# huggingface/parler-tts

Measured on NVIDIA H100. Metric: audio codec tokens/sec (all codebooks), higher is better.
Workload: dtype bf16

## Files before the change

### parler_tts_b200/csrc/sample_core.cuh

```cuda
#pragma once
#include <cfloat>
#include "common.cuh"
#include "kernels.h"

namespace ptts {

__device__ __forceinline__ uint32_t fkey(float f) {
  uint32_t u = __float_as_uint(f);
  return (u & 0x80000000u) ? ~u : (u | 0x80000000u);
}

__device__ __forceinline__ void philox_round(uint32_t (&c)[4], uint32_t k0, uint32_t k1) {
  const uint32_t hi0 = __umulhi(0xD2511F53u, c[0]), lo0 = 0xD2511F53u * c[0];
  const uint32_t hi1 = __umulhi(0xCD9E8D57u, c[2]), lo1 = 0xCD9E8D57u * c[2];
  c[0] = hi1 ^ c[1] ^ k0; c[1] = lo1; c[2] = hi0 ^ c[3] ^ k1; c[3] = lo0;
}
__device__ __forceinline__ float philox_uniform(uint64_t seed, uint32_t row, uint32_t col) {
  uint32_t c[4] = {row, col, 0x5054u, 0x5453u};
  uint32_t k0 = (uint32_t)seed, k1 = (uint32_t)(seed >> 32);
#pragma unroll
  for (int i = 0; i < 10; i++) { philox_round(c, k0, k1); k0 += 0x9E3779B9u; k1 += 0xBB67AE85u; }
  return (float)(c[0] >> 8) * (1.0f / 16777216.0f);
}


constexpr int SMP_WARPS = 8;
constexpr int SMP_THREADS = SMP_WARPS * 32;

constexpr int SMP_MAX_ROWS = 3;
struct SmpScratch {
  float f[2][SMP_MAX_ROWS][SMP_WARPS];
  int i[2][SMP_MAX_ROWS][SMP_WARPS];
  int z[2][SMP_MAX_ROWS][SMP_WARPS];
};
__device__ __forceinline__ SmpScratch& smp_scratch() {
  __shared__ SmpScratch sc;
  return sc;
}
constexpr int SMP_BAN_WORDS = 9 * SMP_THREADS / 32;
__device__ __forceinline__ uint32_t (&smp_bans())[SMP_MAX_ROWS][SMP_BAN_WORDS] {
  __shared__ uint32_t ban[SMP_MAX_ROWS][SMP_BAN_WORDS];
  return ban;
}
struct SmpSeq {
  int last[SMP_MAX_ROWS][PTTS_SEQ_BIAS_MAX];
  float bias[PTTS_SEQ_BIAS_MAX];
};
__device__ __forceinline__ SmpSeq& smp_seq() {
  __shared__ SmpSeq sq;
  return sq;
}
__device__ __forceinline__ bool bitmap_has(const uint32_t* __restrict__ bits, int i) { return (__ldg(bits + (i >> 5)) >> (i & 31)) & 1u; }

template <int ITEMS, int R, bool EXT = false, bool RAGGED = false>
__device__ __forceinline__ void sample_rows_cta(const SampleArgs& p, const ptts_gen_params& g, const int64_t* __restrict__ forced,
                                                int row0, int stride, int n_rows, int cur_len, ptts_sampling_ext x = {},
                                                SampleOut o = {}, ptts_logits_ext lx = {}) {
  static_assert(R >= 1 && R <= SMP_MAX_ROWS, "rows per pass");
  SmpScratch& sc = smp_scratch();
  float (&s_f)[2][SMP_MAX_ROWS][SMP_WARPS] = sc.f;
  int (&s_i)[2][SMP_MAX_ROWS][SMP_WARPS] = sc.i;
  int (&s_z)[2][SMP_MAX_ROWS][SMP_WARPS] = sc.z;
  const int tid = threadIdx.x, lane = tid & 31, warp = tid >> 5;
  int buf = 0;
  auto cta_sum_i = [&](int (&v)[R]) {
#pragma unroll
    for (int r = 0; r < R; r++) {
      const int w = __reduce_add_sync(0xffffffffu, v[r]);
      if (lane == 0) s_i[buf][r][warp] = w;
    }
    __syncthreads();
#pragma unroll
    for (int r = 0; r < R; r++) {
      int a = 0;
#pragma unroll
      for (int w = 0; w < SMP_WARPS; w++) a += s_i[buf][r][w];
      v[r] = a;
    }
    buf ^= 1;
  };
  auto cta_sum_f = [&](float (&v)[R]) {
#pragma unroll
    for (int r = 0; r < R; r++) {
      const float w = warp_sum(v[r]);
      if (lane == 0) s_f[buf][r][warp] = w;
    }
    __syncthreads();
#pragma unroll
    for (int r = 0; r < R; r++) {
      float a = 0.f;
#pragma unroll
      for (int w = 0; w < SMP_WARPS; w++) a += s_f[buf][r][w];
      v[r] = a;
    }
    buf ^= 1;
  };
  auto cta_max_f = [&](float (&v)[R]) {
#pragma unroll
    for (int r = 0; r < R; r++) {
      const float w = warp_max(v[r]);
      if (lane == 0) s_f[buf][r][warp] = w;
    }
    __syncthreads();
#pragma unroll
    for (int r = 0; r < R; r++) {
      float a = s_f[buf][r][0];
#pragma unroll
      for (int w = 1; w < SMP_WARPS; w++) a = fmaxf(a, s_f[buf][r][w]);
      v[r] = a;
    }
    buf ^= 1;
  };

  int row[R];
  bool valid[R];
  int col[R];
  float v[R][ITEMS];
#pragma unroll
  for (int r = 0; r < R; r++) {
    row[r] = row0 + r * stride;
    valid[r] = row[r] < n_rows;
    col[r] = cur_len - ((RAGGED && valid[r]) ? row_shift(p.shift, row[r] / p.K) : 0);
#pragma unroll
    for (int j = 0; j < ITEMS; j++) {
      const int i = tid + SMP_THREADS * j;
      v[r][j] = (valid[r] && i < p.V) ? __ldcg(p.logits + (size_t)row[r] * p.V + i) : -INFINITY;
    }
  }
  auto out_row = [&](float* base, int r) -> float* {
    const int step = cur_len - (g.input_len > 1 ? g.input_len : 1);
    if (base == nullptr || !valid[r] || step < o.first_step || step - o.first_step >= o.n_steps) return nullptr;
    return base + (int64_t)(step - o.first_step) * o.step_stride + (int64_t)row[r] * p.V;
  };
  if constexpr (EXT) {
#pragma unroll
    for (int r = 0; r < R; r++) {
      if (float* dst = out_row(o.logits, r)) {
#pragma unroll
        for (int j = 0; j < ITEMS; j++) {
          const int i = tid + SMP_THREADS * j;
          if (i < p.V) __stcs(dst + i, v[r][j]);
// ... 34 lines not shown
#pragma unroll
  for (int r = 0; r < R; r++) {
    forced_bos[r] = EXT && lx.forced_bos_token_id >= 0 && col[r] == 1;
    const int sh = cur_len - col[r];
    const int begin = lx.begin_index - sh + ((sh > 0 && g.input_len - sh == 1 && lx.forced_bos_token_id >= 0) ? 1 : 0);
    begin_sup[r] = EXT && lx.begin_suppress != nullptr && col[r] == begin;
  }
  if constexpr (EXT) {
    if (lx.n_seq > 0) {
      SmpSeq& sq = smp_seq();
#pragma unroll
      for (int r = 0; r < R; r++) {
        for (int q = tid; q < lx.n_seq; q += SMP_THREADS) {
          const int32_t* e = lx.seq + q * (1 + PTTS_SEQ_BIAS_MAX_LEN);
          const int len = e[0];
          int last = -1;
          if (valid[r] && len >= 2 && len <= PTTS_SEQ_BIAS_MAX_LEN && len <= col[r]) {
            const int64_t* h = p.raw_ids + (size_t)row[r] * p.raw_ld + col[r] - (len - 1);
            bool match = true;
            for (int t = 0; t < len - 1 && match; t++) match = h[t] == e[1 + t];
            if (match) last = e[len];
          }
          sq.last[r][q] = last;
          if (r == 0) sq.bias[q] = lx.seq_bias[q];
        }
      }
      __syncthreads();
    }
  }
#pragma unroll
  for (int r = 0; r < R; r++) {
    const int b = row[r] / p.K, k = row[r] - b * p.K;
    bool mask_eos = false;
    if (cur_len - (g.input_len > 1 ? g.input_len : 1) < g.min_new_tokens) mask_eos = true;
    const bool mask_min = mask_eos;
    bool mask_par = false;
    if (valid[r]) {
      const int par = cur_len & 1;
      int fu = p.first_unf[par * p.B + b];
      const int es = __ldcg(p.eos_seen + fu);
      if (es > 0 && es <= col[r] && fu < b * p.K + p.K - 1) fu++;
      if (k == 0 && tid == 0) p.first_unf[(par ^ 1) * p.B + b] = fu;
      if (row[r] > fu) mask_eos = mask_par = true;
    }
    if (seq_bias || forced_bos[r] || forced_eos || decay || (EXT && lx.remove_invalid_values)) {
      const float mult = decay ? __ldg(lx.decay + cur_len) : 0.f;
#pragma unroll
      for (int j = 0; j < ITEMS; j++) {
        const int i = tid + SMP_THREADS * j;
        if (i >= p.V) continue;
        float y = v[r][j];
        if (seq_bias) {
          float bs = lx.bias1 != nullptr ? __fadd_rn(0.f, __ldg(lx.bias1 + i)) : 0.f;
          for (int q = 0; q < lx.n_seq; q++)
            if (smp_seq().last[r][q] == i) bs = __fadd_rn(bs, smp_seq().bias[q]);
          y = __fadd_rn(y, bs);
        }
        if (bans && ((smp_bans()[r][i >> 5] >> (i & 31)) & 1u)) y = -INFINITY;
        if (mask_min && i == p.eos) y = -INFINITY;
        if (forced_bos[r]) y = (i == lx.forced_bos_token_id) ? 0.f : -INFINITY;
        if (forced_eos) y = (i == lx.forced_eos_token_id) ? 0.f : -INFINITY;
        if (lx.remove_invalid_values) y = (y != y) ? 0.f : (y == INFINITY ? FLT_MAX : (y == -INFINITY ? -FLT_MAX : y));
        if (decay) y = __fadd_rn(y, i == p.eos ? __fmul_rn(fabsf(y), mult) : 0.f);
        if (lx.suppress != nullptr && bitmap_has(lx.suppress, i)) y = -INFINITY;
        if (begin_sup[r] && bitmap_has(lx.begin_suppress, i)) y = -INFINITY;
        if (mask_par && i == p.eos) y = -INFINITY;
        if (g.suppress_special && i >= g.codebook_size) y = -INFINITY;
        v[r][j] = y;
      }
      continue;
    }
#pragma unroll
    for (int j = 0; j < ITEMS; j++) {
      const int i = tid + SMP_THREADS * j;
      if (mask_eos && i == p.eos) v[r][j] = -INFINITY;
      if (g.suppress_special && i >= g.codebook_size) v[r][j] = -INFINITY;
      if constexpr (EXT) {
        if (bans && ((smp_bans()[r][i >> 5] >> (i & 31)) & 1u)) v[r][j] = -INFINITY;
        if (i < p.V && lx.suppress != nullptr && bitmap_has(lx.suppress, i)) v[r][j] = -INFINITY;
        if (i < p.V && begin_sup[r] && bitmap_has(lx.begin_suppress, i)) v[r][j] = -INFINITY;
      }
    }
  }
  int tok[R];
#pragma unroll
  for (int r = 0; r < R; r++) tok[r] = 0;
  const bool renorm = EXT && lx.renormalize_logits;
  float n_max[R], n_log[R];
  if (g.do_sample) {
    if (g.temperature != 1.0f) {
#pragma unroll
      for (int r = 0; r < R; r++)
#pragma unroll
        for (int j = 0; j < ITEMS; j++) v[r][j] = v[r][j] / g.temperature;
    }
    if (g.top_k > 0) {
      const int kk = g.top_k < p.V ? g.top_k : p.V;
      uint32_t key[R][ITEMS];
      uint32_t th[R];
#pragma unroll
      for (int r = 0; r < R; r++) {
        th[r] = 0;
#pragma unroll
        for (int j = 0; j < ITEMS; j++) key[r][j] = (tid + SMP_THREADS * j < p.V) ? fkey(v[r][j]) : 0u;
      }
      for (int bit = 31; bit >= 0; bit--) {
        int cnt[R];
#pragma unroll
        for (int r = 0; r < R; r++) {
          const uint32_t cand = th[r] | (1u << bit);
          cnt[r] = 0;
#pragma unroll
          for (int j = 0; j < ITEMS; j++) cnt[r] += (key[r][j] >= cand) ? 1 : 0;
        }
        cta_sum_i(cnt);
#pragma unroll
        for (int r = 0; r < R; r++)
          if (cnt[r] >= kk) th[r] |= (1u << bit);
      }
#pragma unroll
      for (int r = 0; r < R; r++)
#pragma unroll
        for (int j = 0; j < ITEMS; j++)
          if (fkey(v[r][j]) < th[r]) v[r][j] = -INFINITY;
    }
    float m[R];
#pragma unroll
    for (int r = 0; r < R; r++) {
      m[r] = -INFINITY;
#pragma unroll
      for (int j = 0; j < ITEMS; j++) m[r] = fmaxf(m[r], v[r][j]);
    }
    cta_max_f(m);
    float e[R][ITEMS];
    float s[R];
#pragma unroll
    for (int r = 0; r < R; r++) {
      s[r] = 0.f;
#pragma unroll
      for (int j = 0; j < ITEMS; j++) { e[r][j] = expf(v[r][j] - m[r]); s[r] += e[r][j]; }
    }
    cta_sum_f(s);
    if (g.top_p < 1.0f) {
      uint32_t th[R];
#pragma unroll
      for (int r = 0; r < R; r++) th[r] = 0;
      for (int bit = 31; bit >= 0; bit--) {
        float c[R];
#pragma unroll
        for (int r = 0; r < R; r++) {
          const uint32_t cand = th[r] | (1u << bit);
          c[r] = 0.f;
#pragma unroll
          for (int j = 0; j < ITEMS; j++) c[r] += (fkey(v[r][j]) <= cand) ? e[r][j] : 0.f;
        }
        cta_sum_f(c);
#pragma unroll
        for (int r = 0; r < R; r++)
          if (c[r] <= (1.0f - g.top_p) * s[r]) th[r] |= (1u << bit);
      }
#pragma unroll
      for (int r = 0; r < R; r++) {
        const uint32_t kmax = fkey(m[r]);
        s[r] = 0.f;
#pragma unroll
        for (int j = 0; j < ITEMS; j++) {
          const uint32_t key = fkey(v[r][j]);
          if (key <= th[r] && key != kmax) { v[r][j] = -INFINITY; e[r][j] = 0.f; }
          s[r] += e[r][j];
        }
      }
      cta_sum_f(s);
    }
    if constexpr (EXT) {
      auto drop_where = [&](auto&& remove) {
#pragma unroll
        for (int r = 0; r < R; r++) {
          const float inv = 1.0f / s[r];
          s[r] = 0.f;
#pragma unroll
          for (int j = 0; j < ITEMS; j++) {
            if (remove(r, j, inv)) { v[r][j] = -INFINITY; e[r][j] = 0.f; }
            s[r] += e[r][j];
          }
        }
        cta_sum_f(s);
      };
      auto entropy = [&](float (&ent)[R], float (&lse)[R]) {
#pragma unroll
        for (int r = 0; r < R; r++) {
          lse[r] = m[r] + logf(s[r]);
          ent[r] = 0.f;
#pragma unroll
          for (int j = 0; j < ITEMS; j++)
            if (v[r][j] > -INFINITY) { const float lp = v[r][j] - lse[r]; ent[r] += lp * expf(lp); }
        }
        cta_sum_f(ent);
#pragma unroll
        for (int r = 0; r < R; r++) ent[r] = -ent[r];
      };
      if (x.min_p > 0.f)
        drop_where([&](int r, int j, float inv) { return e[r][j] * inv < x.min_p * inv; });
      if (x.typical_p < 1.0f) {
        float ent[R], lse[R];
        entropy(ent, lse);
        uint32_t key[R][ITEMS], th[R];
#pragma unroll
        for (int r = 0; r < R; r++) {
          th[r] = 0;
#pragma unroll
          for (int j = 0; j < ITEMS; j++) key[r][j] = fkey(v[r][j] > -INFINITY ? fabsf(lse[r] - v[r][j] - ent[r]) : INFINITY);
        }
        for (int bit = 31; bit >= 0; bit--) {
          float c[R];
#pragma unroll
          for (int r = 0; r < R; r++) {
            const uint32_t cand = th[r] | (1u << bit);
            c[r] = 0.f;
#pragma unroll
            for (int j = 0; j < ITEMS; j++) c[r] += (key[r][j] <= cand) ? e[r][j] : 0.f;
          }
          cta_sum_f(c);
#pragma unroll
          for (int r = 0; r < R; r++)
            if (c[r] < x.typical_p * s[r]) th[r] |= (1u << bit);
        }
        drop_where([&](int r, int j, float) { return th[r] != 0xffffffffu && key[r][j] > th[r] + 1u; });
      }
      if (x.epsilon_cutoff > 0.f)
        drop_where([&](int r, int j, float inv) { return e[r][j] * inv < x.epsilon_cutoff && v[r][j] < m[r]; });
      if (x.eta_cutoff > 0.f) {
        float ent[R], lse[R];
        entropy(ent, lse);
        drop_where([&](int r, int j, float inv) {
          return e[r][j] * inv < fminf(x.eta_cutoff, sqrtf(x.eta_cutoff) * expf(-ent[r])) && v[r][j] < m[r];
        });
      }
    }
    float target[R], carry[R];
    int found[R], last_nz[R];
#pragma unroll
    for (int r = 0; r < R; r++) {
      target[r] = philox_uniform(g.seed, (uint32_t)(row[r] + g.row_base), (uint32_t)col[r]) * s[r];
      carry[r] = 0.f; found[r] = -1; last_nz[r] = -1;
    }
#pragma unroll
    for (int j = 0; j < ITEMS; j++) {
      float x[R];
#pragma unroll
      for (int r = 0; r < R; r++) {
        x[r] = e[r][j];
#pragma unroll
        for (int o = 1; o < 32; o <<= 1) {
          const float y = __shfl_up_sync(0xffffffffu, x[r], o);
          if (lane >= o) x[r] += y;
        }
        if (lane == 31) s_f[buf][r][warp] = x[r];
      }
      __syncthreads();
      float tot[R];
#pragma unroll
      for (int r = 0; r < R; r++) {
        float base = carry[r];
        tot[r] = carry[r];
#pragma unroll
        for (int w = 0; w < SMP_WARPS; w++) {
          const float tw = s_f[buf][r][w];
          if (w < warp) base += tw;
          tot[r] += tw;
        }
        const float cum = base + x[r];
        const unsigned hit = __ballot_sync(0xffffffffu, cum > target[r] && e[r][j] > 0.f);
        const unsigned nz = __ballot_sync(0xffffffffu, e[r][j] > 0.f);
        if (lane == 0) {
          s_i[buf][r][warp] = hit ? SMP_THREADS * j + 32 * warp + (__ffs(hit) - 1) : 0x7fffffff;
          s_z[buf][r][warp] = nz ? SMP_THREADS * j + 32 * warp + (31 - __clz(nz)) : -1;
        }
      }
      __syncthreads();
#pragma unroll
      for (int r = 0; r < R; r++) {
        int first = 0x7fffffff, lastz = -1;
#pragma unroll
        for (int w = 0; w < SMP_WARPS; w++) { first = min(first, s_i[buf][r][w]); lastz = max(lastz, s_z[buf][r][w]); }
        if (found[r] < 0 && first != 0x7fffffff) found[r] = first;
        if (lastz >= 0) last_nz[r] = lastz;
        carry[r] = tot[r];
      }
      buf ^= 1;
    }
#pragma unroll
    for (int r = 0; r < R; r++) tok[r] = found[r] >= 0 ? found[r] : last_nz[r];
    if constexpr (EXT) {
#pragma unroll
      for (int r = 0; r < R; r++) {
        if (tok[r] < 0) tok[r] = 0;
        n_max[r] = m[r];
        n_log[r] = logf(s[r]);
      }
    }
  } else {
#pragma unroll
    for (int r = 0; r < R; r++) {
      float m = -INFINITY;
      int mi = 0x7fffffff;
#pragma unroll
      for (int j = 0; j < ITEMS; j++) {
        const int i = tid + SMP_THREADS * j;
        if (i < p.V && (v[r][j] > m || (v[r][j] == m && i < mi))) { m = v[r][j]; mi = i; }
      }
#pragma unroll
      for (int o = 16; o > 0; o >>= 1) {
        const float om = __shfl_xor_sync(0xffffffffu, m, o);
        const int oi = __shfl_xor_sync(0xffffffffu, mi, o);
        if (om > m || (om == m && oi < mi)) { m = om; mi = oi; }
      }
      if (lane == 0) { s_f[buf][r][warp] = m; s_i[buf][r][warp] = mi; }
    }
    __syncthreads();
#pragma unroll
    for (int r = 0; r < R; r++) {
      float m = s_f[buf][r][0];
      int mi = s_i[buf][r][0];
#pragma unroll
      for (int w = 1; w < SMP_WARPS; w++) {
        const float om = s_f[buf][r][w];
        const int oi = s_i[buf][r][w];
        if (om > m || (om == m && oi < mi)) { m = om; mi = oi; }
      }
      tok[r] = mi;
    }
    buf ^= 1;
    if (renorm) {
#pragma unroll
      for (int r = 0; r < R; r++) {
        n_max[r] = -INFINITY;
#pragma unroll
        for (int j = 0; j < ITEMS; j++) n_max[r] = fmaxf(n_max[r], v[r][j]);
      }
      cta_max_f(n_max);
#pragma unroll
      for (int r = 0; r < R; r++) {
        n_log[r] = 0.f;
#pragma unroll
        for (int j = 0; j < ITEMS; j++) n_log[r] += expf(v[r][j] - n_max[r]);
      }
      cta_sum_f(n_log);
#pragma unroll
      for (int r = 0; r < R; r++) n_log[r] = logf(n_log[r]);
    }
  }
  if (renorm) {
#pragma unroll
    for (int r = 0; r < R; r++)
#pragma unroll
      for (int j = 0; j < ITEMS; j++) v[r][j] = (v[r][j] - n_max[r]) - n_log[r];
  }
#pragma unroll
  for (int r = 0; r < R; r++) {
    if (!valid[r]) continue;
#pragma unroll
    for (int j = 0; j < ITEMS; j++) {
      const int i = tid + SMP_THREADS * j;
      if (i < p.V) p.scores[(size_t)row[r] * p.V + i] = v[r][j];
    }
    if constexpr (EXT) {
      if (float* dst = out_row(o.scores, r)) {
#pragma unroll
        for (int j = 0; j < ITEMS; j++) {
          const int i = tid + SMP_THREADS * j;
          if (i < p.V) __stcs(dst + i, v[r][j]);
        }
      }
    }
  }
  int my_tok = 0, my_row = 0, my_col = 0;
  bool my_valid = false;
#pragma unroll
  for (int r = 0; r < R; r++)
    if (tid == r) { my_tok = tok[r]; my_row = row[r]; my_valid = valid[r]; my_col = col[r]; }
  if (tid < R && my_valid) {
    const int b = my_row / p.K, k = my_row - b * p.K;
    int t = my_tok;
    if (forced != nullptr) t = (int)forced[my_row];
    if (!t_unf) t = p.pad;
    p.raw_ids[(size_t)my_row * p.raw_ld + my_col] = t;
    if (t == p.eos && t_es == 0) p.eos_seen[my_row] = my_col + 1;
    const int new_len = cur_len + 1;
    const int done = (t == p.eos) || (new_len >= g.max_length);
    const int still_unfinished = t_unf && !done;
    p.unfinished[my_row] = still_unfinished;
    const int sh = cur_len - my_col;
    const int Lb = g.max_length - sh, nb = g.input_len - sh;
    int nxt = t;
    if (Lb >= 2 * p.K - 1) {
      const bool is_bos = my_col <= k;
      const bool is_pad = (my_col - k) >= (Lb - p.K + 1);
      if (is_bos || is_pad) nxt = (is_bos ? p.bos : 0) + (is_pad ? p.pad : 0);
      else if (nb > 1 && my_col - nb < k) nxt = (int)p.prefix_cells[(size_t)my_row * (p.K - 1) + (my_col - nb)];
    }
    p.cur_ids[my_row] = nxt;
    if (still_unfinished) atomicAdd(&p.ctrl->n_unfinished, 1);
  }
  __syncthreads();
}

template <int ITEMS>
__device__ __forceinline__ void sample_row_cta(const SampleArgs& p, const ptts_gen_params& g, const int64_t* __restrict__ forced,
                                               int row, int cur_len) {
  sample_rows_cta<ITEMS, 1>(p, g, forced, row, 0, row + 1, cur_len);
}

template <int ITEMS, bool RAGGED = false>
__device__ __forceinline__ void sample_all_rows_cta(const SampleArgs& p, const ptts_gen_params& g, int cta, int n_ctas, int n_rows, int cur_len) {
  if (n_rows <= n_ctas) {
    if (cta < n_rows) sample_rows_cta<ITEMS, 1, false, RAGGED>(p, g, nullptr, cta, n_ctas, n_rows, cur_len);
  } else {
    for (int row0 = cta; row0 < n_rows; row0 += 3 * n_ctas) sample_rows_cta<ITEMS, 3, false, RAGGED>(p, g, nullptr, row0, n_ctas, n_rows, cur_len);
  }
}

}
```

### parler_tts_b200/csrc/step2.cu

```cuda
#include "attn_core.cuh"
#include "common.cuh"
#include "kernels.h"
#include "ln_stats.cuh"
#include "sample_core.cuh"
#include "ptx.cuh"
#include "step.h"
#include "step_common.cuh"
#include <type_traits>

namespace ptts {
namespace cl {

constexpr int C = 2;
constexpr int V = 8;
constexpr int THREADS = 256;
constexpr int ROWS = 32;
constexpr int HROWS = 8;
constexpr int ATT_SMEM = attn_decode_smem_per_warp<bf16>();
constexpr int PROF_STRIDE = 16;
constexpr int QMAX = 6;
constexpr int OFF_STATS = 256, OFF_PART = 512, OFF_RES = 2560, OFF_CVEC = 3584;
constexpr int HDR = 5632;
constexpr int WB_BYTES = 65536;
constexpr int R_OFF = HDR + 2 * WB_BYTES;
constexpr int R_BYTES = 92160;
constexpr int QKV_OFF = R_BYTES - 2048;
constexpr int SMEM_BYTES = R_OFF + R_BYTES;
static_assert(SMEM_BYTES + 1024 <= 227 * 1024, "cluster step kernel shared memory");
static_assert(ROWS * (1024 / 2 + 8) * 2 + V * (256 + ROWS * 34 * 4) <= R_BYTES, "fc1 plan");
static_assert(HROWS * (1024 / 2 + 8) * 2 + V * C * (32 + 4 * 96 * 4) <= QKV_OFF, "QKV plan");
constexpr int ATT_STAGE = 2 * 32 * HD * 2;
constexpr int ATT_REST = ATT_SMEM - ATT_STAGE;
constexpr int ATT_S0_QKV = 34 * 1024;
constexpr int ATT_S0_QC = QKV_OFF - V * ATT_STAGE;
constexpr int ATT_S0_WB = WB_BYTES - ATT_STAGE;
static_assert(HROWS * (1024 / 2 + 8) * 2 + V * C * (32 + 4 * 96 * 4) <= ATT_S0_QKV && ATT_S0_QKV + 6 * ATT_STAGE <= QKV_OFF, "attention plan: QKV stages in R");
static_assert(HROWS * (1024 / 2 + 8) * 2 + V * C * (32 + 4 * 32 * 4) <= ATT_S0_QC, "attention plan: q_cross stages in R");
static_assert(2 * ATT_REST <= ATT_S0_QC && 2 * ATT_REST <= ATT_S0_QKV && 6 * ATT_REST <= ATT_S0_WB, "attention plan: second stages");
static_assert(6 * 8 * (1024 / 2) * 2 <= ATT_S0_WB && 16384 + 4 * 128 * 4 <= ATT_S0_WB, "attention plan: QKV weight jobs, out-proj job + pair merge");
static_assert(ROWS * (4096 / 4 + 8) * 2 + V * (256 + ROWS * 8 * 4) <= R_BYTES, "fc2 plan");

__device__ __forceinline__ void mbar_wait(uint64_t* bar, uint32_t parity, int what) {
  uint32_t ok, spins = 0;
  do {
    ok = mbar_try_wait_cluster(bar, parity);
    if (!ok && ++spins > (1u << 22)) { printf("ptts: cluster step mbarrier timeout (cta %d, barrier kind %d)\n", (int)blockIdx.x, what); __trap(); }
  } while (!ok);
}
__device__ __forceinline__ void st_async(uint32_t dst_cluster_addr, float v, uint32_t bar_cluster_addr) {
  asm volatile("st.async.shared::cluster.mbarrier::complete_tx::bytes.b32 [%0], %1, [%2];"
               ::"r"(dst_cluster_addr), "r"(__float_as_uint(v)), "r"(bar_cluster_addr) : "memory");
}
__device__ __forceinline__ void st_async(uint32_t dst_cluster_addr, float2 v, uint32_t bar_cluster_addr) {
  asm volatile("st.async.shared::cluster.mbarrier::complete_tx::bytes.v2.f32 [%0], {%1, %2}, [%3];"
               ::"r"(dst_cluster_addr), "f"(v.x), "f"(v.y), "r"(bar_cluster_addr) : "memory");
}
__device__ __forceinline__ uint32_t mapa(uint32_t addr, uint32_t rank) { uint32_t r; asm volatile("mapa.shared::cluster.u32 %0, %1, %2;" : "=r"(r) : "r"(addr), "r"(rank)); return r; }
__device__ __forceinline__ uint32_t cluster_rank() { uint32_t r; asm volatile("mov.u32 %0, %%cluster_ctarank;" : "=r"(r)); return r; }
__device__ __forceinline__ void cluster_arrive() { asm volatile("barrier.cluster.arrive.release.aligned;" ::: "memory"); }
__device__ __forceinline__ void cluster_wait() { asm volatile("barrier.cluster.wait.acquire.aligned;" ::: "memory"); }
__device__ __forceinline__ void cluster_arrive_reuse() { asm volatile("barrier.cluster.arrive.relaxed.aligned;" ::: "memory"); }

__host__ __device__ __forceinline__ int kslice(int kt) { return (kt & 7) >> 2; }
__host__ __device__ __forceinline__ int klocal(int kt) { return ((kt >> 3) << 2) | (kt & 3); }
__host__ __device__ __forceinline__ int kglobal(int rank, int lk) { return ((lk >> 2) << 3) | (rank << 2) | (lk & 3); }

template <int QN, int MT, bool STATS, bool ACC = false>
__device__ __forceinline__ void mma_slice(float (&out)[2][6][4], RowStatFrag& rst, const bf16* xs, int apitch, const uint4* wb, int KT, int kt0,
                                          int kt_end, int lrow, int lcol) {
  float acc[MT][QN][4];
#pragma unroll
  for (int a = 0; a < MT; a++)
#pragma unroll
    for (int j = 0; j < QN; j++)
#pragma unroll
      for (int e = 0; e < 4; e++) acc[a][j][e] = ACC ? out[a][j][e] : 0.f;
  for (int kt = kt0; kt < kt_end; kt += 4) {
    uint32_t a[MT][2][4];
#pragma unroll
    for (int mt = 0; mt < MT; mt++)
#pragma unroll
      for (int j = 0; j < 2; j++) ldmatrix_x4(a[mt][j], xs + (size_t)(mt * 16 + lrow) * apitch + kt * 32 + j * 16 + lcol);
    if (STATS) {
#pragma unroll
      for (int mt = 0; mt < MT; mt++) { row_stat_mma(rst, mt, a[mt][0]); row_stat_mma(rst, mt, a[mt][1]); }
    }
#pragma unroll
    for (int j = 0; j < QN; j++) {
      const uint4 w = wb[((size_t)j * KT + kt) * 32];
#pragma unroll
      for (int mt = 0; mt < MT; mt++) {
        mma_bf16_16816(acc[mt][j], a[mt][0], w.x, w.y);
        mma_bf16_16816(acc[mt][j], a[mt][1], w.z, w.w);
      }
    }
  }
#pragma unroll
  for (int mt = 0; mt < MT; mt++)
#pragma unroll
    for (int j = 0; j < QN; j++)
#pragma unroll
      for (int e = 0; e < 4; e++) out[mt][j][e] = acc[mt][j][e];
}

enum { PH_QKV = 0, PH_O = 1, PH_QC = 2, PH_OC = 3, PH_FC1 = 4, PH_FC2 = 5 };
constexpr int JOBS_PER_LAYER = 9;
constexpr int QKV_JOBS = 4;

__device__ __forceinline__ bool weight_job(const StepParams& p, int j, int cta, int rank, const char*& src, uint32_t& bytes) {
  const int nl = JOBS_PER_LAYER * p.L;
  if (j < nl) {
    const int l = j / JOBS_PER_LAYER, jl = j - JOBS_PER_LAYER * l;
    const int ph = jl < QKV_JOBS ? 0 : jl - (QKV_JOBS - 1);
    const int64_t idx = (ph == PH_QKV || ph == PH_QC) ? (int64_t)(cta >> 3) * C + rank : (int64_t)cta;
    const int64_t sz = p.lay.cp_slice[ph];
    bytes = (uint32_t)(ph == PH_QKV ? sz / QKV_JOBS : sz);
    src = p.blob + p.lay.layer0 + p.lay.layer_stride * l + p.lay.cp[ph] + idx * sz + (ph == PH_QKV ? jl * (sz / QKV_JOBS) : 0);
    return true;
  }
  const int task = cta + (int)gridDim.x * (j - nl);
  const int ntasks = p.K * p.V / 32;
  if (task >= ntasks) return false;
  bytes = (uint32_t)(4 * p.H * 16);
  src = p.blob + p.lay.heads + (int64_t)task * bytes;
  return true;
}

template <int ITEMS, bool RAGGED>
__global__ void __launch_bounds__(THREADS, 1) decode_step_cluster_kernel(const __grid_constant__ StepParams p) {
  extern __shared__ __align__(128) unsigned char smem[];
  Ctrl* ctrl = p.sa.ctrl;
  if (p.prof != nullptr && blockIdx.x == 0 && threadIdx.x == 0) p.prof[(size_t)(6 * p.L + 2) * PROF_STRIDE + 3] = clock64();
  if (ctrl->active == 0) return;
  int cur_len = ctrl->cur_len;
  const unsigned gen = (unsigned)ctrl->launch_gen;
  int pos = p.P + cur_len - 1;
  const int tid = threadIdx.x, warp = tid >> 5, lane = tid & 31;
  const int H = p.H, F = p.F, B = p.B;
  const int rank = (int)cluster_rank(), peer = rank ^ 1;
  const int cta = (int)blockIdx.x;
  const int cluster = cta >> 1;
  const int head = cluster >> 2, rblk = cluster & 3;
  const int Ks = H / C, KsF = F / 4;
  const int pitch = Ks + 8, pitchF = KsF + 8;
  const int qe = F / p.nh / 64;
  const int dgrp = warp & 1, e4 = warp >> 1;

  uint64_t* abar = reinterpret_cast<uint64_t*>(smem);
  uint64_t* wbar = abar + 1;
  uint64_t* xbar = abar + 3;
  uint64_t* attbars = reinterpret_cast<uint64_t*>(smem + 128);
  float* stats = reinterpret_cast<float*>(smem + OFF_STATS);
  float* part = reinterpret_cast<float*>(smem + OFF_PART);
  float* res_s = reinterpret_cast<float*>(smem + OFF_RES);
  float* cvec = reinterpret_cast<float*>(smem + OFF_CVEC);
  unsigned char* Rg = smem + R_OFF;
  const uint32_t peer_xbar = mapa(smem_u32(xbar), (uint32_t)peer);
  uint32_t par_a = 0, par_w = 0, par_x = 0, att_parity = 0;

  if (tid == 0) {
    mbar_init<1>(abar); mbar_init<1>(&wbar[0]); mbar_init<1>(&wbar[1]); mbar_init<1>(xbar);
    asm volatile("fence.mbarrier_init.release.cluster;" ::: "memory");
  }
  attention_decode_init_warp(attbars + 2 * warp, lane);
  cluster_arrive(); cluster_wait();
  unsigned* const bar_ctr = p.bar + (gen & 1u);
  unsigned bar_target = 0u;
  if (cta == 0 && tid == 0) p.bar[(gen + 1u) & 1u] = 0u;

  const char* blob = p.blob;
  long long* const prof0 = (p.prof != nullptr && cta == 0) ? p.prof : nullptr;
  long long* prof = prof0;
  prof_mark(prof, 0);

  auto issue_weight_job = [&](int j) {
    const char* src; uint32_t bytes;
    if (!weight_job(p, j, cta, rank, src, bytes)) return;
    mbar_expect_tx(&wbar[j & 1], bytes);
    bulk_g2s_evict_first(smem + HDR + (j & 1) * WB_BYTES, src, bytes, &wbar[j & 1]);
  };
  __shared__ int s_next_active;
  const int n_steps = (p.do_sample_phase && p.n_steps > 1 && prof0 == nullptr) ? p.n_steps : 1;
  int unfinished_prev = 0;
#pragma unroll 1
  for (int it = 0; it < n_steps; it++) {
  pos = p.P + cur_len - 1;
  prof = prof0;
  cluster_arrive_reuse();
  if (tid == 0) { issue_weight_job(0); issue_weight_job(1); }

  bf16* const x_img = p.cl_x;
  bf16* const a_img = p.cl_attn;
  bf16* const h_img = p.cl_h;
  const int x_slice_elems = ROWS * pitch, h_slice_elems = ROWS * pitchF;
  auto h_offset = [&](int n) {
    const int lk = klocal(n >> 5), kq = KsF >> 5;
    return (size_t)(2 * kslice(n >> 5) + lk / kq) * h_slice_elems + (lk % kq) * 32 + (n & 31);
  };
  const int xo_slice = kslice(cta >> 2), xo_col = klocal(cta >> 2) * 32 + (cta & 3) * 8;

  {
    const int row = tid >> 3, f = tid & 7, n = cta * 8 + f;
    const float v = row < B ? embed_value(p, row, n, row_pos<RAGGED>(p, row, pos)) : 0.f;
    res_s[row * 8 + f] = v;
    x_img[(size_t)xo_slice * x_slice_elems + row * pitch + xo_col + f] = __float2bfloat16_rn(v);
  }
  prof_mark(prof, 6);
  auto request_slice = [&](const bf16* img_slice, uint32_t bytes) {
    fence_proxy_async_smem();
    mbar_expect_tx(abar, bytes);
    bulk_g2s(Rg, img_slice, bytes, abar);
  };
  auto slice_of = [&](int sub, const bf16*& img, uint32_t& bytes) {
    if (sub == PH_QKV || sub == PH_QC) { img = x_img + (size_t)rank * x_slice_elems + (size_t)(HROWS * rblk) * pitch; bytes = (uint32_t)(HROWS * pitch * 2); }
    else if (sub == PH_O || sub == PH_OC) { img = a_img + (size_t)rank * x_slice_elems; bytes = (uint32_t)(x_slice_elems * 2); }
    else if (sub == PH_FC1) { img = x_img + (size_t)rank * x_slice_elems; bytes = (uint32_t)(x_slice_elems * 2); }
    else { img = h_img + (size_t)(2 * rank) * h_slice_elems; bytes = (uint32_t)(h_slice_elems * 2); }
  };
  {
    const bf16* nimg; uint32_t nbytes;
    slice_of(PH_QKV, nimg, nbytes);
    bar_target = grid_sync(bar_ctr, bar_target, -1, false, nullptr, [&]() { request_slice(nimg, nbytes); });
  }
  prof_mark(prof, 7);

  const int lrow = (lane & 7) + ((lane >> 3) & 1) * 8, lcol = (lane >> 4) * 8;
  const int g = lane >> 2, t4 = lane & 3;
  const int n_phases = 6 * p.L;

  const int att_row = HROWS * rblk + 4 * rank + (warp >> 1);
  const int att_slice = kslice(2 * head), att_col = klocal(2 * head) * 32;

#pragma unroll 1
  for (int ph = 0; ph < n_phases; ph++) {
    const int l = ph / 6, sub = ph - 6 * l;
    prof = prof0 ? prof0 + (size_t)(ph + 1) * PROF_STRIDE : nullptr;
    prof_mark(prof, 0);
    const char* lb = blob + p.lay.layer0 + p.lay.layer_stride * l;
    const bool rowpart = (sub == PH_QKV || sub == PH_QC);
    const bool has_ln = (sub == PH_QKV || sub == PH_QC || sub == PH_FC1);
    const int q = (sub == PH_QKV) ? 6 : (sub == PH_QC ? 2 : (sub == PH_FC1 ? qe : 1));
    const int Nc = 4 * q * 8;
    const int KT = (sub == PH_FC2 ? KsF : Ks) >> 5;
    const int apitch = (sub == PH_FC2) ? pitchF : pitch;
    const int act_bytes = (rowpart ? HROWS : ROWS) * apitch * 2;
    const int RS = (q == 1) ? 8 : 8 * q + 2;
    const int blk = rowpart ? 32 + 4 * 16 * q * 4 : 256 + ROWS * RS * 4;
    unsigned char* const recv = Rg + ((act_bytes + 127) & ~127);
    const uint32_t peer_recv = mapa(smem_u32(recv), (uint32_t)peer);
    const uint32_t xbytes = 4u * (rowpart ? V * 4 * 16 * q + V / 2 * 4 * 2 : V / C * (ROWS * 8 * q + (has_ln ? ROWS * 2 : 0)));
    auto put = [&](int d, uint32_t off, auto v) {
      if (d == rank) *reinterpret_cast<decltype(v)*>(recv + off) = v;
      else st_async(peer_recv + off, v, peer_xbar);
    };
    const int j0 = JOBS_PER_LAYER * l + (sub == 0 ? 0 : sub + QKV_JOBS - 1);
    if (tid == 0) mbar_expect_tx(xbar, xbytes);

    auto att_stage0 = [&]() -> unsigned char* {
      if (sub == PH_QC) return Rg + ATT_S0_QC + warp * ATT_STAGE;
      return warp < 6 ? Rg + ATT_S0_QKV + warp * ATT_STAGE : smem + HDR + (warp - 6) * WB_BYTES + ATT_S0_WB;
    };
    if (rowpart && att_row < B)
      attention_decode_request<bf16>(decode_attn_args(p, l, pos, sub == PH_QC), att_row, head, row_pos<RAGGED>(p, att_row, pos), att_stage0(),
                                     attbars + 2 * warp, lane, warp & 1, 2);

    float cv1 = 0.f, cv2 = 0.f;
    if (has_ln) {
      const float* c1; int ntot;
      if (sub == PH_QKV) { c1 = reinterpret_cast<const float*>(lb + p.lay.c_qkv); ntot = p.qkv_rows; }
      else if (sub == PH_QC) { c1 = reinterpret_cast<const float*>(lb + p.lay.c_qc); ntot = H; }
// ... 132 lines not shown
#pragma unroll
        for (int sv = 0; sv < V; sv++) {
          const float* bp = reinterpret_cast<const float*>(recv + (size_t)sv * blk + 256) + row * RS + f;
          const float2 a = *reinterpret_cast<const float2*>(bp), b2 = *reinterpret_cast<const float2*>(bp + 2);
          v[0] += a.x; v[1] += a.y; v[2] += b2.x; v[3] += b2.y;
        }
#pragma unroll
        for (int e = 0; e < 4; e++) v[e] = apply_act(DT<bf16>::rnd(ln_rstd * (v[e] - ln_mean * cvec[f + e]) + cvec[256 + f + e]), p.act);
        uint2 pk;
        pk.x = att_pack(v[0], v[1]); pk.y = att_pack(v[2], v[3]);
        *reinterpret_cast<uint2*>(h_img + h_offset(cta * 32 + f) + row * pitchF) = pk;
      } else if (row < B) {
        for (int i = 0; i < q; i++) {
          const int f = f0 + 8 * i;
          float v = 0.f;
#pragma unroll
          for (int sv = 0; sv < V; sv++) v += reinterpret_cast<const float*>(recv + (size_t)sv * blk + 256)[row * RS + f];
          if (sub == PH_FC1) {
            v = ln_rstd * (v - ln_mean * cvec[f]) + cvec[256 + f];
            v = apply_act(DT<bf16>::rnd(v), p.act);
            h_img[h_offset(cta * 8 * q + f) + row * pitchF] = __float2bfloat16_rn(v);
          } else {
            v = DT<bf16>::rnd(res_s[row * 8 + f] + DT<bf16>::rnd(v));
            res_s[row * 8 + f] = v;
            x_img[(size_t)xo_slice * x_slice_elems + row * pitch + xo_col + f] = __float2bfloat16_rn(v);
          }
        }
      }
    } else {
      bf16* qkv_s = reinterpret_cast<bf16*>(Rg + QKV_OFF);
      auto gather = [&](auto jw_tag) {
        constexpr int JW = decltype(jw_tag)::value, NC = 4 * JW, QCW = 2 * JW;
        for (int idx = tid; idx < 4 * NC; idx += THREADS) {
          const int r4 = idx / NC, col = idx - r4 * NC;
          const int u = col / JW, cw = (u >> 1) * JW + (col - u * JW);
          float S1 = 0.f, S2 = 0.f;
#pragma unroll
          for (int e = 0; e < V; e++) {
            const float2 x = *reinterpret_cast<const float2*>(recv + (size_t)(8 * (e >> 2) + 2 * (e & 3)) * blk + r4 * 8);
            S1 += x.x; S2 += x.y;
          }
          const float ln_mean = S1 / (float)H;
          const float ln_rstd = rsqrtf(fmaxf(S2 / (float)H - ln_mean * ln_mean, 0.f) + p.eps);
          float v = 0.f;
#pragma unroll
          for (int e = 0; e < V; e++)
            v += reinterpret_cast<const float*>(recv + (size_t)(8 * (e >> 2) + 2 * (e & 3) + (u & 1)) * blk + 32)[r4 * QCW + cw];
          v = ln_rstd * (v - ln_mean * cvec[col]) + cvec[256 + col];
          qkv_s[idx] = __float2bfloat16_rn(v);
        }
      };
      if (sub == PH_QKV) gather(std::integral_constant<int, 48>{}); else gather(std::integral_constant<int, 16>{});
      static_assert(HD == 64, "QKV: 2 x 2 units of 6 n-tiles (q|k|v of a head), q_cross: 2 x 2 units of 2 n-tiles");
    }
    prof_mark(prof, 4);
    __syncthreads();
    cluster_arrive_reuse();

    if (rowpart) {
      if (att_row < B) {
        AttnArgs att = decode_attn_args(p, l, pos, sub == PH_QC);
        const bf16* qkv_s = reinterpret_cast<const bf16*>(Rg + QKV_OFF);
        const int row_base = HROWS * rblk + 4 * rank;
        const bf16* qbase = qkv_s - (size_t)row_base * Nc - (size_t)head * HD;
        att.q = qbase; att.ldq = Nc;
        att.ldo = pitch;
        att.out = a_img + (size_t)att_slice * x_slice_elems + att_col - (size_t)head * HD;
        if (sub == PH_QKV) { att.knew = qbase; att.vnew = qbase; att.ldkv = Nc; att.k_col0 = HD; att.v_col0 = 2 * HD; }
        unsigned char* wb0 = smem + HDR;
        unsigned char* held = wb0 + ((sub == PH_QKV ? j0 + 1 : j0) & 1) * WB_BYTES;
        unsigned char* other = wb0 + ((sub == PH_QKV ? j0 : j0 + 1) & 1) * WB_BYTES;
        unsigned char* rest = warp < 2 ? Rg + (size_t)warp * ATT_REST : held + (size_t)(warp - 2) * ATT_REST;
        float* xr = reinterpret_cast<float*>(other + 16384) + (warp >> 1) * 128;
        prof_mark(prof, 10);
        attention_decode_sweep<bf16>(att, att_row, head, row_pos<RAGGED>(p, att_row, pos), att_stage0(), rest, attbars + 2 * warp, lane, att_parity, warp & 1, 2, xr, (warp >> 1) + 1,
                                     true, tid == 0 ? prof : nullptr);
      }
      prof_mark(prof, 5);
    }
    prof_mark(prof, 6);
    if (p.prof != nullptr && l == p.L / 2 && tid == 0) {
      unsigned long long ns;
      asm volatile("mov.u64 %0, %%globaltimer;" : "=l"(ns));
      p.prof[(size_t)(n_phases + 4) * PROF_STRIDE + sub * (int)gridDim.x + cta] = (long long)ns;
    }

    const bool last = (ph + 1 == n_phases);
    const bf16* nimg; uint32_t nbytes;
    if (last) { nimg = x_img; nbytes = (uint32_t)(C * x_slice_elems * 2); }
    else slice_of((sub + 1) % 6, nimg, nbytes);
    const int held_job = sub == PH_QKV ? j0 + QKV_JOBS + 1 : (sub == PH_QC || sub == PH_OC) ? j0 + 2 : -1;
    bar_target = grid_sync(bar_ctr, bar_target, ph, false, nullptr, [&]() {
      request_slice(nimg, nbytes);
      if (held_job >= 0) issue_weight_job(held_job);
    });
    prof_mark(prof, 7);
  }
  cluster_wait();

  prof = prof0 ? prof0 + (size_t)(n_phases + 1) * PROF_STRIDE : nullptr;
  prof_mark(prof, 0);
  {
    const int ntasks = p.K * p.V / 32;
    const float* c1 = reinterpret_cast<const float*>(blob + p.lay.c_heads);
    const float* c2 = c1 + p.K * p.V;
    mbar_wait(abar, par_a, 3);
    par_a ^= 1u;
    const bf16* xs = reinterpret_cast<const bf16*>(Rg);
    const int KTH = H >> 5;
    auto ktile = [&](int kt) { return xs + (size_t)kslice(kt) * x_slice_elems + klocal(kt) * 32; };
    {
      RowStatFrag rst;
      row_stat_zero(rst);
      for (int kt = warp; kt < KTH; kt += 8) {
        const bf16* sl = ktile(kt);
#pragma unroll
        for (int mt = 0; mt < 2; mt++)
#pragma unroll
          for (int j = 0; j < 2; j++) {
            uint32_t a[4];
            ldmatrix_x4(a, sl + (size_t)(mt * 16 + lrow) * pitch + j * 16 + lcol);
            row_stat_mma(rst, mt, a);
          }
      }
      row_stat_store(rst, part, warp, lane);
      __syncthreads();
      row_stat_finalize(part, H, ROWS, p.eps, stats);
      __syncthreads();
    }
    prof_mark(prof, 1);
    constexpr int HRS = 40;
    int job = JOBS_PER_LAYER * p.L;
    for (int task = cta; task < ntasks; task += (int)gridDim.x, job++) {
      mbar_wait(&wbar[job & 1], (par_w >> (job & 1)) & 1u, 4);
      par_w ^= 1u << (job & 1);
      float acc[2][4][4];
#pragma unroll
      for (int a = 0; a < 2; a++)
#pragma unroll
        for (int j = 0; j < 4; j++)
#pragma unroll
          for (int e = 0; e < 4; e++) acc[a][j][e] = 0.f;
      unsigned char* wbuf = smem + HDR + (job & 1) * WB_BYTES;
      const uint4* wb = reinterpret_cast<const uint4*>(wbuf) + lane;
      for (int kt = warp; kt < KTH; kt += 8) {
        const bf16* sl = ktile(kt);
        uint32_t a[2][2][4];
#pragma unroll
        for (int mt = 0; mt < 2; mt++)
#pragma unroll
          for (int j = 0; j < 2; j++) ldmatrix_x4(a[mt][j], sl + (size_t)(mt * 16 + lrow) * pitch + j * 16 + lcol);
#pragma unroll
        for (int j = 0; j < 4; j++) {
          const uint4 w = wb[((size_t)j * KTH + kt) * 32];
#pragma unroll
          for (int mt = 0; mt < 2; mt++) {
            mma_bf16_16816(acc[mt][j], a[mt][0], w.x, w.y);
            mma_bf16_16816(acc[mt][j], a[mt][1], w.z, w.w);
          }
        }
      }
      __syncthreads();
      float* red = reinterpret_cast<float*>(wbuf);
#pragma unroll
      for (int mt = 0; mt < 2; mt++)
#pragma unroll
        for (int j = 0; j < 4; j++) {
          float* base = red + ((size_t)warp * 32 + mt * 16 + g) * HRS + j * 8 + 2 * t4;
          *reinterpret_cast<float2*>(base) = make_float2(acc[mt][j][0], acc[mt][j][1]);
          *reinterpret_cast<float2*>(base + 8 * HRS) = make_float2(acc[mt][j][2], acc[mt][j][3]);
        }
      __syncthreads();
      {
        const int er = tid >> 3, ec = tid & 7;
        if (er < B) {
          const float mean = stats[2 * er], rstd = stats[2 * er + 1];
#pragma unroll
          for (int j = 0; j < 4; j++) {
            const int cidx = j * 8 + ec, n = task * 32 + cidx;
            float v = 0.f;
#pragma unroll
            for (int w = 0; w < 8; w++) v += red[((size_t)w * 32 + er) * HRS + cidx];
            p.logits[(size_t)er * p.K * p.V + n] = DT<bf16>::rnd(rstd * (v - mean * c1[n]) + c2[n]);
          }
        }
      }
      __syncthreads();
      if (tid == 32) {
        fence_proxy_async_smem();
        issue_weight_job(job + 2);
      }
    }
  }
  prof_mark(prof, 6);
  bar_target = grid_sync(bar_ctr, bar_target, n_phases, true);
  prof = prof0 ? prof0 + (size_t)(n_phases + 2) * PROF_STRIDE : nullptr;
  prof_mark(prof, 0);
  if (p.do_sample_phase) {
    const ptts_gen_params gp = *p.sa.gen;
    const int BK = B * p.K;
    sample_phase<ITEMS, RAGGED>(p.sa, gp, BK, cur_len);
    prof_mark(prof, 1);
    bar_target = grid_sync(bar_ctr, bar_target, n_phases + 1, true, nullptr, [&]() {
      const int tot = *reinterpret_cast<volatile int*>(&ctrl->n_unfinished);
      s_next_active = (tot - unfinished_prev > 0) ? 1 : 0;
      unfinished_prev = tot;
    });
    prof_mark(prof, 2);
  }
  bool go_on = false;
  if (p.do_sample_phase) {
    const int act = s_next_active;
    if (cta == 0 && tid == 0) {
      ctrl->cur_len = cur_len + 1;
      ctrl->active = act;
      ctrl->steps_run += 1;
    }
    go_on = act != 0;
    cur_len += 1;
  }
  if (!go_on) break;
  }
  if (cta == 0 && tid == 0) {
    if (p.do_sample_phase) ctrl->n_unfinished = 0;
    ctrl->launch_gen = (int)(gen + 1u);
  }
}

__global__ void cluster_pack_kernel(const uint4* __restrict__ src, uint4* __restrict__ dst, int ph, int nh, int ntc, int kts, int KT_src) {
  const int64_t tile = blockIdx.x;
  const int ktl = (int)(tile % kts);
  const int j = (int)((tile / kts) % ntc);
  const int slice = (int)(tile / ((int64_t)kts * ntc));
  const int rank = slice & 1, owner = slice >> 1;
  int n_tile;
  if (ph == PH_QKV) n_tile = (j >> 3) * (nh * 8) + owner * 8 + (j & 7);
  else n_tile = owner * ntc + j;
  const int kt = kglobal(rank, ktl);
  dst[tile * 32 + threadIdx.x] = src[((int64_t)n_tile * KT_src + kt) * 32 + threadIdx.x];
}

}

int cluster_pack_layer(const DecoderLayout& L, char* layer, cudaStream_t st) {
  for (int ph = 0; ph < 6; ph++) {
    const ClusterPhase cp = cluster_phase(L, ph);
    const int64_t tiles = (int64_t)cp.owners * cl::C * cp.nt * cp.kt;
    cl::cluster_pack_kernel<<<(unsigned)tiles, 32, 0, st>>>(reinterpret_cast<const uint4*>(layer + cp.mat),
                                                            reinterpret_cast<uint4*>(layer + L.cp[ph]), ph, L.nh, cp.nt, cp.kt, cp.kt_src);
  }
  PTTS_LAUNCH_CHECK();
  return PTTS_OK;
}

static const void* cluster_kernel_fn(const StepParams& p) {
  const bool rg = p.sa.shift != nullptr;
  if (p.sample_items <= 1) return rg ? (const void*)cl::decode_step_cluster_kernel<1, true> : (const void*)cl::decode_step_cluster_kernel<1, false>;
  if (p.sample_items <= 5) return rg ? (const void*)cl::decode_step_cluster_kernel<5, true> : (const void*)cl::decode_step_cluster_kernel<5, false>;
  return rg ? (const void*)cl::decode_step_cluster_kernel<9, true> : (const void*)cl::decode_step_cluster_kernel<9, false>;
}

static void cluster_launch_config(const StepParams& p, cudaLaunchConfig_t& cfg, cudaLaunchAttribute* at, cudaStream_t st) {
  cfg = cudaLaunchConfig_t{};
  cfg.gridDim = dim3((unsigned)(4 * p.nh * cl::C));
  cfg.blockDim = dim3(cl::THREADS);
  cfg.dynamicSmemBytes = cl::SMEM_BYTES;
  cfg.stream = st;
  at[0].id = cudaLaunchAttributeClusterDimension;
  at[0].val.clusterDim.x = cl::C; at[0].val.clusterDim.y = 1; at[0].val.clusterDim.z = 1;
  at[1].id = cudaLaunchAttributeCooperative;
  at[1].val.cooperative = 1;
  cfg.attrs = at;
  cfg.numAttrs = 2;
}

bool cluster_step_available(const StepParams& p) {
  const void* fn = cluster_kernel_fn(p);
  static bool told = false;
  auto why = [&](const char* what, cudaError_t e, int n) {
    if (!told) fprintf(stderr, "ptts_b200: cluster step kernel not used (%s: %s, %d co-resident clusters of %d, need %d); the one-CTA-per-SM step kernel runs instead\n",
                       what, cudaGetErrorString(e), n, cl::C, 4 * p.nh);
    told = true;
    cudaGetLastError();
    return false;
// ... 24 lines not shown
```

### parler_tts_b200/csrc/step_common.cuh

```cuda
#pragma once
#include "attn_core.cuh"
#include "common.cuh"
#include "sample_core.cuh"
#include "step.h"

namespace ptts {

template <bool RAGGED>
__device__ __forceinline__ int row_pos(const StepParams& p, int b, int pos) { return RAGGED ? pos - row_shift(p.sa.shift, b) : pos; }

__device__ __forceinline__ float embed_value(const StepParams& p, int row, int col, int pos) {
  const bf16* tables = reinterpret_cast<const bf16*>(p.blob + p.lay.embed);
  float v = 0.f;
#pragma unroll 1
  for (int k0 = 0; k0 < p.K; k0 += 8) {
    float ev[8];
#pragma unroll
    for (int k = 0; k < 8; k++)
      if (k0 + k < p.K) ev[k] = __bfloat162float(tables[((size_t)(k0 + k) * (p.V + 1) + p.sa.cur_ids[row * p.K + k0 + k]) * p.H + col]);
#pragma unroll
    for (int k = 0; k < 8; k++)
      if (k0 + k < p.K) v = (k0 + k == 0) ? ev[k] : DT<bf16>::rnd(v + ev[k]);
  }
  if (!p.rope) v = DT<bf16>::rnd(v + __bfloat162float(reinterpret_cast<const bf16*>(p.blob + p.lay.pos)[(size_t)pos * p.H + col]));
  return v;
}

__device__ __forceinline__ AttnArgs decode_attn_args(const StepParams& p, int l, int pos, bool cross) {
  AttnArgs a{};
  a.ctrl = nullptr; a.B = p.B; a.nh = p.nh; a.q_len = 1;
  a.past_from_ctrl = 0; a.past_len = pos; a.prefix = p.P;
  a.rope = p.rope; a.rope_cos = p.blob + p.lay.rope_cos; a.rope_sin = p.blob + p.lay.rope_sin; a.scale = p.scale;
  if (!cross) {
    char* kc = p.self_kv + p.self_layer_stride * l;
    a.kcache = kc; a.vcache = kc + (size_t)p.B * p.nkv * p.Tmax * HD * 2;
    a.kv_b_stride = (int64_t)p.nkv * p.Tmax * HD; a.kv_h_stride = (int64_t)p.Tmax * HD; a.kv_t_stride = HD; a.kv_b_div = 1;
    a.key_mask = p.prompt_mask; a.mask_len = p.P; a.mask_ld = p.P;
    a.nkv = p.nkv; a.cross = 0; a.kv_len = 0; a.kv_capacity = p.Tmax;
  } else {
    char* ck = p.cross_kv + p.cross_layer_stride * l;
    a.kcache = ck; a.vcache = ck + (size_t)(p.B / p.takes) * p.nckv * p.S * HD * 2;
    a.kv_b_stride = (int64_t)p.nckv * p.S * HD; a.kv_h_stride = (int64_t)p.S * HD; a.kv_t_stride = HD; a.kv_b_div = p.takes;
    a.key_mask = p.enc_mask; a.mask_len = p.S; a.mask_ld = p.S;
    a.nkv = p.nckv; a.cross = 1; a.kv_len = p.S; a.kv_capacity = p.S;
  }
  return a;
}

template <int ITEMS, bool RAGGED>
__device__ __noinline__ void sample_phase(const SampleArgs& sa, const ptts_gen_params& gp, int BK, int cur_len) {
  sample_all_rows_cta<ITEMS, RAGGED>(sa, gp, (int)blockIdx.x, (int)gridDim.x, BK, cur_len);
}

}
```

Measured before the change: 254,400.

## Exit sampling scan early, prefetch LM-head scale vectors, batch embedding id loads, add profiling

The cumulative-probability scan in sampling now exits once every valid row has found its token, so later chunks are not scanned. The LM-head epilogue loads its c1/c2 scale vectors into registers before waiting on the weight barrier. Embedding lookup now loads 16 codebook ids up front, reads the positional embedding early, and then gathers the tables. Per-step profiling stamps are also added and multi-step runs are allowed while profiling; the extra stamp branches add a little overhead when profiling is off.

Result: faster. 257,600, median of 6 (+1.3%).

```diff
diff --git a/parler_tts_b200/csrc/sample_core.cuh b/parler_tts_b200/csrc/sample_core.cuh
--- a/parler_tts_b200/csrc/sample_core.cuh
+++ b/parler_tts_b200/csrc/sample_core.cuh
@@ -55,8 +55,9 @@
 template <int ITEMS, int R, bool EXT = false, bool RAGGED = false>
 __device__ __forceinline__ void sample_rows_cta(const SampleArgs& p, const ptts_gen_params& g, const int64_t* __restrict__ forced,
                                                 int row0, int stride, int n_rows, int cur_len, ptts_sampling_ext x = {},
-                                                SampleOut o = {}, ptts_logits_ext lx = {}) {
+                                                SampleOut o = {}, ptts_logits_ext lx = {}, long long* prof = nullptr) {
   static_assert(R >= 1 && R <= SMP_MAX_ROWS, "rows per pass");
+  auto stamp = [&](int slot) { if (prof != nullptr && threadIdx.x == 0) prof[slot] = clock64(); };
   SmpScratch& sc = smp_scratch();
   float (&s_f)[2][SMP_MAX_ROWS][SMP_WARPS] = sc.f;
   int (&s_i)[2][SMP_MAX_ROWS][SMP_WARPS] = sc.i;
@@ -257,6 +258,7 @@
       }
     }
   }
+  stamp(4);
   int tok[R];
 #pragma unroll
   for (int r = 0; r < R; r++) tok[r] = 0;
@@ -298,6 +300,7 @@
 #pragma unroll
         for (int j = 0; j < ITEMS; j++)
           if (fkey(v[r][j]) < th[r]) v[r][j] = -INFINITY;
+      stamp(5);
     }
     float m[R];
 #pragma unroll
@@ -463,6 +466,10 @@
         carry[r] = tot[r];
       }
       buf ^= 1;
+      bool drawn = true;
+#pragma unroll
+      for (int r = 0; r < R; r++) drawn = drawn && (found[r] >= 0 || !valid[r]);
+      if (drawn) break;
     }
 #pragma unroll
     for (int r = 0; r < R; r++) tok[r] = found[r] >= 0 ? found[r] : last_nz[r];
@@ -525,6 +532,7 @@
       for (int r = 0; r < R; r++) n_log[r] = logf(n_log[r]);
     }
   }
+  stamp(6);
   if (renorm) {
 #pragma unroll
     for (int r = 0; r < R; r++)
@@ -587,12 +595,14 @@
 }
 
 template <int ITEMS, bool RAGGED = false>
-__device__ __forceinline__ void sample_all_rows_cta(const SampleArgs& p, const ptts_gen_params& g, int cta, int n_ctas, int n_rows, int cur_len) {
+__device__ __forceinline__ void sample_all_rows_cta(const SampleArgs& p, const ptts_gen_params& g, int cta, int n_ctas, int n_rows, int cur_len,
+                                                    long long* prof = nullptr) {
   if (n_rows <= n_ctas) {
-    if (cta < n_rows) sample_rows_cta<ITEMS, 1, false, RAGGED>(p, g, nullptr, cta, n_ctas, n_rows, cur_len);
+    if (cta < n_rows) sample_rows_cta<ITEMS, 1, false, RAGGED>(p, g, nullptr, cta, n_ctas, n_rows, cur_len, {}, {}, {}, prof);
   } else {
-    for (int row0 = cta; row0 < n_rows; row0 += 3 * n_ctas) sample_rows_cta<ITEMS, 3, false, RAGGED>(p, g, nullptr, row0, n_ctas, n_rows, cur_len);
-  }
-}
-
-}
+    for (int row0 = cta; row0 < n_rows; row0 += 3 * n_ctas)
+      sample_rows_cta<ITEMS, 3, false, RAGGED>(p, g, nullptr, row0, n_ctas, n_rows, cur_len, {}, {}, {}, prof);
+  }
+}
+
+}
diff --git a/parler_tts_b200/csrc/step2.cu b/parler_tts_b200/csrc/step2.cu
--- a/parler_tts_b200/csrc/step2.cu
+++ b/parler_tts_b200/csrc/step2.cu
@@ -18,6 +18,7 @@
 constexpr int HROWS = 8;
 constexpr int ATT_SMEM = attn_decode_smem_per_warp<bf16>();
 constexpr int PROF_STRIDE = 16;
+__device__ __forceinline__ size_t prof_token_elems(int L) { return (size_t)(6 * L + 4) * PROF_STRIDE + 6 * gridDim.x; }
 constexpr int QMAX = 6;
 constexpr int OFF_STATS = 256, OFF_PART = 512, OFF_RES = 2560, OFF_CVEC = 3584;
 constexpr int HDR = 5632;
@@ -169,9 +170,8 @@
   if (cta == 0 && tid == 0) p.bar[(gen + 1u) & 1u] = 0u;
 
   const char* blob = p.blob;
-  long long* const prof0 = (p.prof != nullptr && cta == 0) ? p.prof : nullptr;
-  long long* prof = prof0;
-  prof_mark(prof, 0);
+  long long* prof0 = nullptr;
+  long long* prof = nullptr;
 
   auto issue_weight_job = [&](int j) {
     const char* src; uint32_t bytes;
@@ -180,12 +180,14 @@
     bulk_g2s_evict_first(smem + HDR + (j & 1) * WB_BYTES, src, bytes, &wbar[j & 1]);
   };
   __shared__ int s_next_active;
-  const int n_steps = (p.do_sample_phase && p.n_steps > 1 && prof0 == nullptr) ? p.n_steps : 1;
+  const int n_steps = (p.do_sample_phase && p.n_steps > 1) ? p.n_steps : 1;
   int unfinished_prev = 0;
 #pragma unroll 1
   for (int it = 0; it < n_steps; it++) {
   pos = p.P + cur_len - 1;
+  if (p.prof != nullptr && cta == 0) prof0 = p.prof + (size_t)it * prof_token_elems(p.L);
   prof = prof0;
+  prof_mark(prof, 0);
   cluster_arrive_reuse();
   if (tid == 0) { issue_weight_job(0); issue_weight_job(1); }
 
@@ -484,7 +486,7 @@
     if (p.prof != nullptr && l == p.L / 2 && tid == 0) {
       unsigned long long ns;
       asm volatile("mov.u64 %0, %%globaltimer;" : "=l"(ns));
-      p.prof[(size_t)(n_phases + 4) * PROF_STRIDE + sub * (int)gridDim.x + cta] = (long long)ns;
+      p.prof[(size_t)it * prof_token_elems(p.L) + (size_t)(n_phases + 4) * PROF_STRIDE + sub * (int)gridDim.x + cta] = (long long)ns;
     }
 
     const bool last = (ph + 1 == n_phases);
@@ -508,6 +510,7 @@
     const float* c2 = c1 + p.K * p.V;
     mbar_wait(abar, par_a, 3);
     par_a ^= 1u;
+    prof_mark(prof, 1);
     const bf16* xs = reinterpret_cast<const bf16*>(Rg);
     const int KTH = H >> 5;
     auto ktile = [&](int kt) { return xs + (size_t)kslice(kt) * x_slice_elems + klocal(kt) * 32; };
@@ -530,12 +533,16 @@
       row_stat_finalize(part, H, ROWS, p.eps, stats);
       __syncthreads();
     }
-    prof_mark(prof, 1);
+    prof_mark(prof, 2);
     constexpr int HRS = 40;
     int job = JOBS_PER_LAYER * p.L;
-    for (int task = cta; task < ntasks; task += (int)gridDim.x, job++) {
+    for (int task = cta, t = 0; task < ntasks; task += (int)gridDim.x, job++, t++) {
+      float hc1[4], hc2[4];
+#pragma unroll
+      for (int j = 0; j < 4; j++) { const int n = task * 32 + j * 8 + (tid & 7); hc1[j] = c1[n]; hc2[j] = c2[n]; }
       mbar_wait(&wbar[job & 1], (par_w >> (job & 1)) & 1u, 4);
       par_w ^= 1u << (job & 1);
+      if (t < 4) prof_mark(prof, 3 + 3 * t);
       float acc[2][4][4];
 #pragma unroll
       for (int a = 0; a < 2; a++)
@@ -562,6 +569,7 @@
           }
         }
       }
+      if (t < 4) prof_mark(prof, 4 + 3 * t);
       __syncthreads();
       float* red = reinterpret_cast<float*>(wbuf);
 #pragma unroll
@@ -583,7 +591,7 @@
             float v = 0.f;
 #pragma unroll
             for (int w = 0; w < 8; w++) v += red[((size_t)w * 32 + er) * HRS + cidx];
-            p.logits[(size_t)er * p.K * p.V + n] = DT<bf16>::rnd(rstd * (v - mean * c1[n]) + c2[n]);
+            p.logits[(size_t)er * p.K * p.V + n] = DT<bf16>::rnd(rstd * (v - mean * hc1[j]) + hc2[j]);
           }
         }
       }
@@ -592,16 +600,17 @@
         fence_proxy_async_smem();
         issue_weight_job(job + 2);
       }
-    }
-  }
-  prof_mark(prof, 6);
+      if (t < 4) prof_mark(prof, 5 + 3 * t);
+    }
+  }
+  prof_mark(prof, 15);
   bar_target = grid_sync(bar_ctr, bar_target, n_phases, true);
   prof = prof0 ? prof0 + (size_t)(n_phases + 2) * PROF_STRIDE : nullptr;
   prof_mark(prof, 0);
   if (p.do_sample_phase) {
     const ptts_gen_params gp = *p.sa.gen;
     const int BK = B * p.K;
-    sample_phase<ITEMS, RAGGED>(p.sa, gp, BK, cur_len);
+    sample_phase<ITEMS, RAGGED>(p.sa, gp, BK, cur_len, prof);
     prof_mark(prof, 1);
     bar_target = grid_sync(bar_ctr, bar_target, n_phases + 1, true, nullptr, [&]() {
       const int tot = *reinterpret_cast<volatile int*>(&ctrl->n_unfinished);
diff --git a/parler_tts_b200/csrc/step_common.cuh b/parler_tts_b200/csrc/step_common.cuh
--- a/parler_tts_b200/csrc/step_common.cuh
+++ b/parler_tts_b200/csrc/step_common.cuh
@@ -10,19 +10,24 @@
 __device__ __forceinline__ int row_pos(const StepParams& p, int b, int pos) { return RAGGED ? pos - row_shift(p.sa.shift, b) : pos; }
 
 __device__ __forceinline__ float embed_value(const StepParams& p, int row, int col, int pos) {
+  constexpr int G = 16;
   const bf16* tables = reinterpret_cast<const bf16*>(p.blob + p.lay.embed);
+  const float pe = p.rope ? 0.f : __bfloat162float(reinterpret_cast<const bf16*>(p.blob + p.lay.pos)[(size_t)pos * p.H + col]);
   float v = 0.f;
 #pragma unroll 1
-  for (int k0 = 0; k0 < p.K; k0 += 8) {
-    float ev[8];
+  for (int k0 = 0; k0 < p.K; k0 += G) {
+    int id[G];
 #pragma unroll
-    for (int k = 0; k < 8; k++)
-      if (k0 + k < p.K) ev[k] = __bfloat162float(tables[((size_t)(k0 + k) * (p.V + 1) + p.sa.cur_ids[row * p.K + k0 + k]) * p.H + col]);
+    for (int k = 0; k < G; k++) id[k] = k0 + k < p.K ? p.sa.cur_ids[row * p.K + k0 + k] : 0;
+    float ev[G];
 #pragma unroll
-    for (int k = 0; k < 8; k++)
+    for (int k = 0; k < G; k++)
+      if (k0 + k < p.K) ev[k] = __bfloat162float(tables[((size_t)(k0 + k) * (p.V + 1) + id[k]) * p.H + col]);
+#pragma unroll
+    for (int k = 0; k < G; k++)
       if (k0 + k < p.K) v = (k0 + k == 0) ? ev[k] : DT<bf16>::rnd(v + ev[k]);
   }
-  if (!p.rope) v = DT<bf16>::rnd(v + __bfloat162float(reinterpret_cast<const bf16*>(p.blob + p.lay.pos)[(size_t)pos * p.H + col]));
+  if (!p.rope) v = DT<bf16>::rnd(v + pe);
   return v;
 }
 
@@ -48,8 +53,8 @@
 }
 
 template <int ITEMS, bool RAGGED>
-__device__ __noinline__ void sample_phase(const SampleArgs& sa, const ptts_gen_params& gp, int BK, int cur_len) {
-  sample_all_rows_cta<ITEMS, RAGGED>(sa, gp, (int)blockIdx.x, (int)gridDim.x, BK, cur_len);
+__device__ __noinline__ void sample_phase(const SampleArgs& sa, const ptts_gen_params& gp, int BK, int cur_len, long long* prof = nullptr) {
+  sample_all_rows_cta<ITEMS, RAGGED>(sa, gp, (int)blockIdx.x, (int)gridDim.x, BK, cur_len, prof);
 }
 
 }
```
